# GaiYu0/dgl-1

Hardware: AMD Instinct MI355X
Metric: edges/sec on update_all g-SpMM (copy_u+sum, feat=128) (higher is better)
Workload: dtype fp32

## Files before the change

### dgl-1_amd/csrc/gspmm.hip

```cpp

#include "gspmm_impl.h"

namespace dglhip {

struct GatEpi {
  const float* a;
  const float* w;
  const float* dz;
  float alpha, lo, hi, scale;
  int apply_exp;
  float* rsum = nullptr;
  int hash_keep = 0;
  uint64_t seed = 0;
  const int64_t* seed_off = nullptr;
  uint32_t thr = 0;
  const float* el = nullptr;
  const float* er = nullptr;
};

__device__ __forceinline__ float gat_slope(const GatEpi& e, float a, int xpos) {
  if (xpos >= 0) return xpos ? 1.0f : e.alpha;
  return e.apply_exp ? (a <= 1.0f ? e.alpha : 1.0f) : (a <= 0.0f ? e.alpha : 1.0f);
}

// ... 441 lines not shown
  if (num_chunks > 0) {
    SumLaunch c{num_chunks, feat_len, elen, indptr, indices, eid, ufeat, efeat, partial,
                nullptr, chunk_beg, chunk_end, false, false, ufeat_ld};
    dispatch_sum(msg_op, false, c, stream);
  }
  if (num_light > 0) {
    SumLaunch l{num_light, feat_len, elen, indptr, indices, eid, ufeat, efeat, out,
                light_rows, nullptr, nullptr, accum,
                stream_output(num_light + num_heavy, feat_len), ufeat_ld};
    dispatch_sum(msg_op, mean, l, stream);
  }
  if (num_heavy > 0) {
    const int64_t blocks = (num_heavy + 3) / 4;
    auto combine = mean ? (accum ? gspmm_combine_kernel<true, true> : gspmm_combine_kernel<true, false>)
                        : (accum ? gspmm_combine_kernel<false, true> : gspmm_combine_kernel<false, false>);
    timed_launch(stream, [&] {
      hipLaunchKernelGGL(combine, grid_1d(blocks), dim3(256), 0, stream, num_heavy, feat_len,
                         indptr, heavy_rows, heavy_chunk_ptr, partial, out);
    });
  }
  API_END();
}

int dglhip_gspmm_items_columns_device(int msg_op, int64_t num_items, int64_t feat_len,
                                      const int32_t* item_rows, const int64_t* item_ptr,
                                      int accumulate, const int32_t* indices, const int64_t* eid,
                                      const float* ufeat, int64_t ufeat_ld, int64_t ufeat_rows,
                                      int items_per_wave, int column_parts, const float* efeat,
                                      int64_t efeat_len, float* out, void* stream_) {
  API_BEGIN();
  hipStream_t stream = static_cast<hipStream_t>(stream_);
  DGLHIP_CHECK(msg_op >= 0 && msg_op <= 3, "unknown msg op " << msg_op);
  DGLHIP_CHECK(num_items >= 0 && feat_len >= 0 && ufeat_rows >= 0, "negative size");
  DGLHIP_CHECK(items_per_wave == 1 || items_per_wave == 2,
               "items_per_wave " << items_per_wave << ": 1 or 2");
  DGLHIP_CHECK(column_parts == 1 || column_parts == 2,
               "column_parts " << column_parts << ": 1 or 2");
  if (num_items == 0 || feat_len == 0) return 0;
  DGLHIP_CHECK(item_rows && item_ptr && indices && out, "null items/indices/out");
  const int64_t elen = check_operands(msg_op, feat_len, ufeat, efeat, efeat_len);
  check_ufeat_ld(ufeat_ld, feat_len);
  SumLaunch a{num_items, feat_len, elen, nullptr, indices, eid, ufeat, efeat,
              out, item_rows, item_ptr, item_ptr + 1, accumulate != 0, false, ufeat_ld,
              ufeat_rows, items_per_wave, items_per_wave == 2 ? column_parts : 1};
  dispatch_sum(msg_op, false, a, stream);
  API_END();
}

int dglhip_gspmm_items_table_device(int msg_op, int64_t num_items, int64_t feat_len,
                                    const int32_t* item_rows, const int64_t* item_ptr,
                                    int accumulate, const int32_t* indices, const int64_t* eid,
                                    const float* ufeat, int64_t ufeat_ld, int64_t ufeat_rows,
                                    int items_per_wave, const float* efeat, int64_t efeat_len,
                                    float* out, void* stream_) {
  return dglhip_gspmm_items_columns_device(msg_op, num_items, feat_len, item_rows, item_ptr,
                                           accumulate, indices, eid, ufeat, ufeat_ld, ufeat_rows,
                                           items_per_wave, 1, efeat, efeat_len, out, stream_);
}

int dglhip_gspmm_items_device(int msg_op, int64_t num_items, int64_t feat_len,
                              const int32_t* item_rows, const int64_t* item_ptr, int accumulate,
                              const int32_t* indices, const int64_t* eid, const float* ufeat,
                              int64_t ufeat_ld, const float* efeat, int64_t efeat_len,
                              float* out, void* stream_) {
  return dglhip_gspmm_items_table_device(msg_op, num_items, feat_len, item_rows, item_ptr,
                                         accumulate, indices, eid, ufeat, ufeat_ld, 0, 1, efeat,
                                         efeat_len, out, stream_);
}

// ... 328 lines not shown
```

### dgl-1_amd/csrc/gspmm_impl.h

```cpp
#pragma once
#include <hip/hip_runtime.h>

#include <algorithm>
#include <cstdint>
#include <initializer_list>
#include <mutex>
#include <vector>

#include "../../include/dgl_hip.h"
#include "common.h"
#include "launch.h"
#include "timing.h"

namespace dglhip {

__host__ __device__ __forceinline__ uint32_t gat_mix32(uint32_t x) {
  x ^= x >> 16;
  x *= 0x7feb352du;
  x ^= x >> 15;
  x *= 0x846ca68bu;
  x ^= x >> 16;
  return x;
}

__host__ __device__ __forceinline__ bool gat_keep(uint64_t seed, int64_t idx, uint32_t thr) {
  const uint64_t i = static_cast<uint64_t>(idx);
  const uint32_t r = gat_mix32(gat_mix32(static_cast<uint32_t>(i) ^ static_cast<uint32_t>(seed)) ^
                               (static_cast<uint32_t>(i >> 32) + static_cast<uint32_t>(seed >> 32) +
                                0x9e3779b9u));
  return r >= thr;
}

static inline uint32_t gat_drop_threshold(float p) {
  const double t = static_cast<double>(p) * 4294967296.0;
  return t >= 4294967295.0 ? 0xffffffffu : static_cast<uint32_t>(t);
}

typedef float f32x2 __attribute__((ext_vector_type(2)));
typedef float f32x4 __attribute__((ext_vector_type(4)));

template <int VEC> struct Vec;
template <> struct Vec<1> {
  typedef float T;
  static __device__ __forceinline__ T zero() { return 0.0f; }
  static __device__ __forceinline__ T splat(float x) { return x; }
  static __device__ __forceinline__ T fma(T a, T b, T c) { return __builtin_fmaf(a, b, c); }
  static __device__ __forceinline__ T max(T a, T b) { return a > b ? a : b; }
};
template <> struct Vec<2> {
  typedef f32x2 T;
  static __device__ __forceinline__ T zero() { return T{0.0f, 0.0f}; }
  static __device__ __forceinline__ T splat(float x) { return T{x, x}; }
  static __device__ __forceinline__ T fma(T a, T b, T c) {
    return T{__builtin_fmaf(a.x, b.x, c.x), __builtin_fmaf(a.y, b.y, c.y)};
  }
};
template <> struct Vec<4> {
  typedef f32x4 T;
  static __device__ __forceinline__ T zero() { return T{0.0f, 0.0f, 0.0f, 0.0f}; }
// ... 385 lines not shown
      const int rb = nmax - k;
      u32x4 v[DEPTH];
#pragma unroll
      for (int j = 0; j < DEPTH; ++j) {
        if (j < rb)
          v[j] = __builtin_amdgcn_raw_buffer_load_b128(table, row_broadcast(ids, j) + lane_off,
                                                       0, 0);
      }
      if (k + DEPTH < nmax) ids = batch_ids(k + DEPTH);
#pragma unroll
      for (int j = 0; j < DEPTH; ++j) {
        if (j < rb) {
          const f32x4 sum = acc + *reinterpret_cast<const f32x4*>(&v[j]);
          acc = k + j < my_n ? sum : acc;
        }
      }
    }
  }
#pragma unroll
  for (int t = 0; t < 4; ++t)
    if (q == t && i0 + t < num_items) store_out<4, ACCUM ? 2 : 4>(out + r[t] * F, f0, acc);
}

template <bool MEAN, bool ACCUM>
__global__ __launch_bounds__(256) void gspmm_combine_kernel(
    int64_t num_heavy, int64_t F, const int64_t* __restrict__ indptr,
    const int32_t* __restrict__ heavy_rows, const int64_t* __restrict__ heavy_chunk_ptr,
    const float* __restrict__ partial, float* __restrict__ out) {
  const int64_t wave = block_linear() * (blockDim.x >> 6) + (threadIdx.x >> 6);
  if (wave >= num_heavy) return;
  const int lane = threadIdx.x & 63;
  const int64_t row = heavy_rows[wave];
  const int64_t c0 = heavy_chunk_ptr[wave], c1 = heavy_chunk_ptr[wave + 1];
  const float deg = static_cast<float>(indptr[row + 1] - indptr[row]);
  for (int64_t f = lane; f < F; f += 64) {
    float acc = (ACCUM && !MEAN) ? out[row * F + f] + partial[c0 * F + f] : partial[c0 * F + f];
    for (int64_t c = c0 + 1; c < c1; ++c) acc += partial[c * F + f];
    if (MEAN && deg > 1.0f) acc = acc / deg;
    if (MEAN && ACCUM) acc = out[row * F + f] + acc;
    out[row * F + f] = acc;
  }
}

__device__ __forceinline__ bool max_takes(float x, float best) {
  return (best == best) & !(x <= best);
}
// ... 130 lines not shown
  if (group < 64 && F >= 16) {
    vec = 1;
    group = 64;
  }
}

struct SumLaunch {
  int64_t num_items, F, elen;
  const int64_t* indptr;
  const int32_t* indices;
  const int64_t* eid;
  const float* ufeat;
  const float* efeat;
  float* out;
  const int32_t* row_order;
  const int64_t* chunk_beg;
  const int64_t* chunk_end;
  bool accumulate;
  bool nt_out = false;
  int64_t ldu = 0;
  int64_t urows = 0;
  int items_per_wave = 1;
  int column_parts = 1;
};

static inline bool stream_output(int64_t rows, int64_t feat_len) {
  return rows * feat_len * int64_t(sizeof(float)) > (int64_t(512) << 20);
}

static inline bool items_pair_applies(const SumLaunch& a) {
  const int64_t ldu = a.ldu ? a.ldu : a.F;
  return a.items_per_wave == 2 && a.F == 128 && a.urows > 0 && ldu % 4 == 0 &&
         reinterpret_cast<uintptr_t>(a.ufeat) % 16 == 0 &&
         reinterpret_cast<uintptr_t>(a.out) % 16 == 0 &&
         a.urows * ldu * int64_t(sizeof(float)) < (int64_t(1) << 32);
}

static inline bool items_columns_applies(const SumLaunch& a) {
  const int64_t ldu = a.ldu ? a.ldu : a.F;
  return a.column_parts == 2 && items_pair_applies(a) &&
         a.urows * ldu * int64_t(sizeof(float)) <= int64_t(0xfffffc00u);
}

static inline void launch_items_columns(const SumLaunch& a, hipStream_t stream) {
  constexpr int DEPTH = 12;
  const int64_t blocks = 2 * ((a.num_items + 15) / 16);
  DGLHIP_CHECK(blocks <= 0x7fffffff, "grid too large: " << blocks);
  const int64_t ldu = a.ldu ? a.ldu : a.F;
  auto kernel = a.accumulate ? gspmm_items_columns_kernel<DEPTH, true>
                             : gspmm_items_columns_kernel<DEPTH, false>;
  timed_launch(stream, [&] {
    hipLaunchKernelGGL(kernel, grid_1d(blocks), dim3(256), 0, stream, a.num_items, ldu,
                       static_cast<uint32_t>(a.urows * ldu * int64_t(sizeof(float))), a.indices,
                       a.ufeat, a.out, a.row_order, a.chunk_beg);
  });
}

static inline void launch_items_pair(const SumLaunch& a, hipStream_t stream) {
  constexpr int DEPTH = 10;
  const int64_t blocks = (a.num_items + 7) / 8;
  DGLHIP_CHECK(blocks <= 0x7fffffff, "grid too large: " << blocks);
  const int64_t ldu = a.ldu ? a.ldu : a.F;
  auto kernel = a.accumulate ? gspmm_items_pair_kernel<DEPTH, true>
                             : gspmm_items_pair_kernel<DEPTH, false>;
  timed_launch(stream, [&] {
    hipLaunchKernelGGL(kernel, grid_1d(blocks), dim3(256), 0, stream, a.num_items, ldu,
                       static_cast<uint32_t>(a.urows * ldu * int64_t(sizeof(float))), a.indices,
                       a.ufeat, a.out, a.row_order, a.chunk_beg);
  });
}

template <int VEC, int GROUP, int MSG, int EM, bool MEAN>
static inline void launch_sum(const SumLaunch& a, hipStream_t stream) {
  constexpr int UNROLL = 16;
  constexpr int ITEMS_PER_BLOCK = 4 * (64 / GROUP);
  const int64_t blocks = (a.num_items + ITEMS_PER_BLOCK - 1) / ITEMS_PER_BLOCK;
  DGLHIP_CHECK(blocks <= 0x7fffffff, "grid too large: " << blocks);
  if (blocks == 0) return;
  const bool chunked = a.chunk_beg != nullptr;
  auto kernel = gspmm_sum_kernel<VEC, GROUP, UNROLL, MSG, EM, MEAN, false, false>;
  if (chunked && a.accumulate)
    kernel = gspmm_sum_kernel<VEC, GROUP, UNROLL, MSG, EM, MEAN, true, true>;
  else if (chunked)
    kernel = gspmm_sum_kernel<VEC, GROUP, UNROLL, MSG, EM, MEAN, true, false>;
  else if (a.accumulate)
    kernel = gspmm_sum_kernel<VEC, GROUP, UNROLL, MSG, EM, MEAN, false, true>;
  constexpr bool POL_OK = MSG == DGLHIP_MSG_COPY_U && VEC == 2 && GROUP == 64 && !MEAN;
  if constexpr (POL_OK) {
    if (chunked && a.row_order && !a.nt_out) {
      if (items_columns_applies(a)) {
        launch_items_columns(a, stream);
        return;
      }
      if (items_pair_applies(a)) {
        launch_items_pair(a, stream);
        return;
      }
      if (a.accumulate)
        kernel = gspmm_sum_kernel<VEC, GROUP, UNROLL, MSG, EM, false, true, true, POL_DEFAULT,
                                  true, 2>;
      else
        kernel = gspmm_sum_kernel<VEC, GROUP, UNROLL, MSG, EM, false, true, false, POL_DEFAULT,
                                  true, 4>;
    } else if (a.nt_out && !a.accumulate) {
      if (chunked)
        kernel = gspmm_sum_kernel<VEC, GROUP, UNROLL, MSG, EM, false, true, false, POL_NT_OUT>;
      else
        kernel = gspmm_sum_kernel<VEC, GROUP, UNROLL, MSG, EM, false, false, false, POL_NT_OUT>;
    }
  }
  timed_launch(stream, [&] {
    hipLaunchKernelGGL(kernel, grid_1d(blocks), dim3(256), 0, stream, a.num_items, a.F, a.elen,
// ... 95 lines not shown
```

### dgl-1_amd/csrc/spmm_plan.cc

```cpp
#include "spmm_plan.h"

#include <hip/hip_runtime.h>

#include <algorithm>
#include <climits>
#include <cmath>
#include <cstdlib>
#include <cstring>
#include <numeric>
#include <string>

#include "../../include/dgl_hip.h"
#include "common.h"

namespace dglhip {

namespace {

constexpr int64_t kRefWaves = 7168;
constexpr int64_t kCriticalMin = 16384;
constexpr int64_t kCutNum = 7168, kCutDen = 12000;
constexpr int64_t kChunkMin = 1024;

void hip_ok(hipError_t e, const char* what) {
  DGLHIP_CHECK(e == hipSuccess, what << ": " << hipGetErrorString(e));
}

std::string env_str(const char* name, const char* dflt) {
  const char* v = std::getenv(name);
  return v ? std::string(v) : std::string(dflt);
}

SpmmPolicy policy_from_env() {
  SpmmPolicy p;
  const std::string rs = env_str("DGLHIP_ROW_SPLIT", "auto");
  if (rs == "auto") p.row_split = -1;
  else if (rs == "off" || rs == "0" || rs.empty() || rs == "none" || rs == "None") p.row_split = 0;
  else p.row_split = std::stoll(rs);
  p.blocked = env_str("DGLHIP_BLOCKED", "auto") != "off";
  p.block_bytes = std::stoll(env_str("DGLHIP_BLOCK_BYTES", "6291456"));
  p.block_min_slots = std::stoll(env_str("DGLHIP_BLOCK_MIN_SLOTS", "12"));
  p.block_max_stretch = std::stod(env_str("DGLHIP_BLOCK_MAX_STRETCH", "3"));
  p.short_rows = env_str("DGLHIP_SHORT_ROWS", "on") != "off";
  p.pad_rows = env_str("DGLHIP_PAD_ROWS", "auto") == "auto";
  p.items_per_wave = env_str("DGLHIP_ITEMS_PER_WAVE", "2") == "1" ? 1 : 2;
  p.column_parts = env_str("DGLHIP_COLUMN_PARTS", "2") == "1" ? 1 : 2;
  return p;
}

std::mutex g_pol_mu;
SpmmPolicy& pol_ref() {
  static SpmmPolicy p = policy_from_env();
  return p;
}

double lines_per_row(int64_t F, int64_t ld) {
  int64_t tot = 0;
  for (int64_t u = 0; u < 32; ++u) {
    const int64_t off = (u * ld * 4) % 128;
    tot += (off + 4 * F + 127) / 128;
  }
  return tot / 32.0;
}

inline int64_t cdiv(int64_t a, int64_t b) { return (a + b - 1) / b; }

inline bool copies_u(int msg) {
  return msg == DGLHIP_MSG_COPY_U || msg == DGLHIP_MSG_COPY_U_BF16;
}
// ... 28 lines not shown
    const char* bb = std::getenv("DGLHIP_SWEEP_BLOCK_BYTES");
    if (bb && std::atoll(bb) >= (int64_t(1) << 20)) q.block_bytes = std::atoll(bb);
    return q;
  }();
  return p;
}
}

SweepPolicy sweep_policy() {
  std::lock_guard<std::mutex> lk(g_pol_mu);
  return sweep_ref();
}

void set_spmm_policy(const SpmmPolicy& p) {
  DGLHIP_CHECK(p.block_bytes > 0 && p.block_min_slots >= 1 && p.block_max_stretch > 0 &&
                   p.block_table_min >= 0 && p.block_table_max >= p.block_table_min &&
                   p.block_max_suffix >= 0 && p.tier_min_rows >= 0 && p.pad_min_bytes >= 0,
               "invalid g-SpMM schedule policy");
  DGLHIP_CHECK(p.row_split >= -1, "row_split: -1 auto, 0 off or a chunk length");
  DGLHIP_CHECK(p.items_per_wave == 1 || p.items_per_wave == 2,
               "items_per_wave " << p.items_per_wave << ": 1 or 2");
  DGLHIP_CHECK(p.column_parts == 1 || p.column_parts == 2,
               "column_parts " << p.column_parts << ": 1 or 2");
  std::lock_guard<std::mutex> lk(g_pol_mu);
  pol_ref() = p;
}

int64_t split_threshold(const SpmmPolicy& p, int64_t nnz, int64_t max_degree, int64_t waves) {
  if (p.row_split == 0) return 0;
  if (p.row_split < 0) {
    const int64_t R = std::max<int64_t>(waves, 2);
    const int64_t t = std::max<int64_t>(4096, nnz * kCutNum / (kCutDen * R));
    return max_degree > std::max<int64_t>(kCriticalMin, nnz / (R / 2)) ? t : 0;
  }
  return max_degree > p.row_split ? p.row_split : 0;
}

int64_t padded_width(int64_t F) {
  int64_t best = F;
  double best_lines = lines_per_row(F, F);
  for (int64_t ld : {cdiv(F, 16) * 16, cdiv(F, 32) * 32}) {
    if (ld > F && ld % 2 == 0) {
      const double l = lines_per_row(F, ld);
      if (l < best_lines * 0.95 && l < lines_per_row(F, best) - 1e-9) {
        best = ld;
        best_lines = l;
// ... 615 lines not shown
};

enum Path { PATH_HOST = 0, PATH_ROWS = 1, PATH_BLOCKED = 2, PATH_MAX_BLOCKED = 3, PATH_SWEEP = 4 };

int g_blocked_mean_add = [] {
  const char* e = std::getenv("DGLHIP_BLOCKED_MEAN_ADD");
  return e && *e ? std::atoi(e) : 1;
}();

inline bool blocked_mean_add() { return g_blocked_mean_add != 0; }

struct Decision {
  Path path = PATH_ROWS;
  std::shared_ptr<BlockedPlan> bp;
  std::shared_ptr<Cuts> cuts;
  std::shared_ptr<SweepPlan> sw;
  bool pad = false;
  int64_t ld = 0;
  int64_t split = 0;
  int64_t ws_pad = 0, ws_vals = 0, ws_map = 0, ws_partial = 0;
  int64_t ws_sums = 0;
  int items_per_wave = 1;
  int column_parts = 1;
  int64_t total() const { return ws_pad + ws_vals + ws_map + ws_partial + ws_sums; }
};

inline int64_t align256(int64_t b) { return (b + 255) / 256 * 256; }

bool pad_rows(const SpmmPolicy& p, int msg, int red, int64_t F, int64_t urows) {
  return p.pad_rows && (msg == DGLHIP_MSG_COPY_U || msg == DGLHIP_MSG_U_MUL_E) &&
         (red == DGLHIP_REDUCE_SUM || red == DGLHIP_REDUCE_MEAN || accum(red)) &&
         urows * F * 4 >= p.pad_min_bytes && padded_width(F) != F;
}

void check_args(const SpmmPlan& plan, const RunArgs& a) {
  DGLHIP_CHECK(a.msg >= 0 && a.msg <= 3, "unknown msg op " << a.msg);
  DGLHIP_CHECK(a.red >= 0 && a.red <= 4, "unknown reduce op " << a.red);
  DGLHIP_CHECK(a.F >= 0, "negative feat_len");
  DGLHIP_CHECK(a.emode >= DGLHIP_EDGE_BY_SLOT && a.emode <= DGLHIP_EDGE_BY_MAP,
               "unknown edge layout " << a.emode);
  DGLHIP_CHECK(a.ldu == 0 || a.ldu == a.F || (a.ldu > a.F && a.ldu % 2 == 0),
               "ufeat_ld " << a.ldu << ": 0, feat_len, or an even width > feat_len");
  DGLHIP_CHECK(a.ldu <= a.F || (a.msg == DGLHIP_MSG_COPY_U || a.msg == DGLHIP_MSG_U_MUL_E),
               "row-strided source rows: copy_u or u_mul_e");
  DGLHIP_CHECK(a.ldu <= a.F || a.red != DGLHIP_REDUCE_MAX, "row-strided source rows: not max");
  const bool use_u = a.msg != DGLHIP_MSG_COPY_E;
// ... 26 lines not shown
  if ((a.red == DGLHIP_REDUCE_SUM || a.red == DGLHIP_REDUCE_MEAN ||
       a.red == DGLHIP_REDUCE_SUM_ACCUM) && a.msg == DGLHIP_MSG_COPY_U &&
      a.ufeat && !a.efeat && !strided && a.F == 128) {
    d.sw = plan.sweep(a.F * 4,
                      a.red == DGLHIP_REDUCE_SUM_ACCUM ? 2 : (a.red == DGLHIP_REDUCE_MEAN ? 1 : 0),
                      s);
    if (d.sw) {
      d.path = PATH_SWEEP;
      return d;
    }
  }
  const bool mean_add = blocked_mean_add() && a.red == DGLHIP_REDUCE_MEAN_ACCUM &&
                        a.msg == DGLHIP_MSG_COPY_U && !a.efeat;
  if ((sumlike || mean_add) && a.ufeat &&
      ((cu && !a.efeat) || (a.msg == DGLHIP_MSG_U_MUL_E && a.efeat))) {
    d.bp = plan.blocked(ld_in * elem, p.block_bytes, s);
    if (d.bp) {
      d.path = PATH_BLOCKED;
      const auto lh = plan.span(s);
      const double slice = static_cast<double>(lh.second - lh.first) * ld_in * elem / d.bp->B;
      const double reach = p.column_parts == 2 ? 3.0 : 1.5;
      d.items_per_wave = p.items_per_wave == 2 && slice <= reach * p.block_bytes ? 2 : 1;
      d.column_parts = d.items_per_wave == 2 ? p.column_parts : 1;
      if (mean_add) d.ws_sums = align256(plan.num_rows() * a.F * 4);
      if (!strided && fp32u && pad_rows(p, a.msg, DGLHIP_REDUCE_SUM, a.F, a.urows)) {
        d.pad = true;
        d.ld = padded_width(a.F);
        d.ws_pad = align256(a.urows * d.ld * 4);
      } else {
        d.ld = strided ? a.ldu : 0;
      }
      if (a.msg == DGLHIP_MSG_U_MUL_E) {
        if (a.elen == 1) d.ws_vals = align256(plan.nnz() * 4);
        if (a.emode == DGLHIP_EDGE_BY_MAP) d.ws_map = align256(plan.nnz() * 8);
      }
      return d;
    }
  }
  if (a.red == DGLHIP_REDUCE_MAX && a.ufeat && !strided && fp32u &&
      (a.msg == DGLHIP_MSG_COPY_U ||
       (a.msg == DGLHIP_MSG_U_MUL_E &&
        (a.emode == DGLHIP_EDGE_BY_SLOT ||
         (a.emode == DGLHIP_EDGE_BY_EID && plan.eid_identity(a.erow, s)))))) {
    d.cuts = plan.cuts(a.F * 4, p.block_bytes, s);
    if (d.cuts) {
      d.path = PATH_MAX_BLOCKED;
// ... 95 lines not shown
    const int64_t* erows = nullptr;
    if (a.msg == DGLHIP_MSG_U_MUL_E) {
      const int64_t* rows = nullptr;
      if (a.emode == DGLHIP_EDGE_BY_SLOT) {
        rows = plan.plan_pos64(bp, s);
      } else if (a.emode == DGLHIP_EDGE_BY_EID) {
        rows = plan.eid_identity(a.erow, s) ? plan.plan_pos64(bp, s)
                                            : plan.plan_eidmap(bp, a.erow, s);
      } else {
        int64_t* m = reinterpret_cast<int64_t*>(ws.take(d.ws_map));
        plan_compose_device(plan.nnz(), bp.pos.data<int32_t>(), a.erow, m, s);
        rows = m;
      }
      if (a.elen == 1) {
        float* v = reinterpret_cast<float*>(ws.take(d.ws_vals));
        plan_gather_vals_device(plan.nnz(), rows, a.efeat, v, s);
        ev = v;
      } else {
        erows = rows;
      }
    }
    for (size_t i = 0; i < bp.launches.size(); ++i) {
      const BlockItems& it = bp.launches[i];
      DGLHIP_CHECK(dglhip_gspmm_items_columns_device(
                       a.msg, it.n_items, a.F, it.rows.data<int32_t>(), it.ptr.data<int64_t>(),
                       (i == 0 && first_writes) ? 0 : 1, bp.indices.data<int32_t>(),
                       ev ? nullptr : erows, static_cast<const float*>(uf), d.ld, a.urows,
                       d.items_per_wave, d.column_parts,
                       ev ? ev : (a.msg == DGLHIP_MSG_U_MUL_E ? a.efeat : nullptr),
                       elen, sums, s) == 0,
                   DGLGetLastError());
    }
    if (a.red == DGLHIP_REDUCE_MEAN) plan_div_degree_device(plan.num_rows(), a.F, plan.indptr(),
                                                            a.out, s);
    if (d.ws_sums) plan_add_mean_device(plan.num_rows(), a.F, plan.indptr(), sums, a.out, s);
    return;
  }
  if (d.path == PATH_MAX_BLOCKED) {
    const Cuts& c = *d.cuts;
    const int64_t* base = c.data.data<int64_t>();
    const int64_t* eid = nullptr;
    for (int64_t b = 0; b + 1 < c.n; ++b) {
      DGLHIP_CHECK(dglhip_gspmm_max_ranges_device(
                       a.msg, plan.num_rows(), a.F, plan.indptr(), base + b * plan.num_rows(),
                       base + (b + 1) * plan.num_rows(), b ? 1 : 0, plan.indices(), eid,
                       static_cast<const float*>(uf), a.efeat, a.elen, a.out, a.arg,
                       plan.row_order(), s) == 0,
                   DGLGetLastError());
    }
    return;
  }
// ... 152 lines not shown
  *accum_per_cu = p.accum_per_cu;
  API_END();
}

int dglhip_spmm_get_policy(DGLHipSpmmPolicy* out) {
  API_BEGIN();
  DGLHIP_CHECK(out != nullptr, "null pointer argument");
  const SpmmPolicy p = spmm_policy();
  out->row_split = p.row_split;
  out->blocked = p.blocked;
  out->short_rows = p.short_rows;
  out->pad_rows = p.pad_rows;
  out->items_per_wave = p.items_per_wave;
  out->block_bytes = p.block_bytes;
  out->block_table_min = p.block_table_min;
  out->block_table_max = p.block_table_max;
  out->block_min_slots = p.block_min_slots;
  out->block_max_stretch = p.block_max_stretch;
  out->block_max_suffix = p.block_max_suffix;
  out->block_min_row_bytes = p.block_min_row_bytes;
  out->tier_min_rows = p.tier_min_rows;
  out->pad_min_bytes = p.pad_min_bytes;
  out->column_parts = p.column_parts;
  out->reserved = 0;
  API_END();
}

int dglhip_spmm_set_policy(const DGLHipSpmmPolicy* in) {
  API_BEGIN();
  DGLHIP_CHECK(in != nullptr, "null pointer argument");
  SpmmPolicy p;
  p.row_split = in->row_split;
  p.blocked = in->blocked != 0;
  p.short_rows = in->short_rows != 0;
  p.pad_rows = in->pad_rows != 0;
  p.items_per_wave = in->items_per_wave;
  p.block_bytes = in->block_bytes;
  p.block_table_min = in->block_table_min;
  p.block_table_max = in->block_table_max;
  p.block_min_slots = in->block_min_slots;
  p.block_max_stretch = in->block_max_stretch;
  p.block_max_suffix = in->block_max_suffix;
  p.block_min_row_bytes = in->block_min_row_bytes;
  p.tier_min_rows = in->tier_min_rows;
  p.pad_min_bytes = in->pad_min_bytes;
  p.column_parts = in->column_parts;
  set_spmm_policy(p);
  API_END();
}

int dglhip_spmm_split_threshold(int64_t nnz, int64_t max_degree, int64_t waves, int64_t* out) {
  API_BEGIN();
  DGLHIP_CHECK(out != nullptr, "null pointer argument");
  *out = split_threshold(spmm_policy(), nnz, max_degree, waves > 0 ? waves : kRefWaves);
  API_END();
}

int dglhip_spmm_padded_width(int64_t feat_len, int64_t* out) {
  API_BEGIN();
  DGLHIP_CHECK(out != nullptr && feat_len >= 1, "bad argument");
  *out = padded_width(feat_len);
  API_END();
}

int dglhip_spmm_plan_create(int device_type, int device_id, int64_t num_rows, int64_t num_cols,
                            int64_t nnz, const int64_t* indptr, const int32_t* indices,
                            const int64_t* host_indptr, const int32_t* row_order, void* stream,
                            DGLHipSpmmPlan* out) {
  API_BEGIN();
// ... 85 lines not shown
```

### dgl-1_amd/csrc/spmm_plan.h

```cpp
#pragma once

#include <hip/hip_runtime.h>

#include <cstdint>
#include <map>
#include <memory>
#include <mutex>
#include <tuple>
#include <vector>

#include "runtime.h"

namespace dglhip {

struct SpmmPolicy {
  int64_t row_split = -1;
  int blocked = 1;
  int short_rows = 1;
  int pad_rows = 1;
  int items_per_wave = 2;
  int64_t block_bytes = 6 << 20;
  int64_t block_table_min = 16 << 20;
  int64_t block_table_max = 256 << 20;
  int64_t block_min_slots = 12;
  double block_max_stretch = 3.0;
  double block_max_suffix = 1.0 / 16;
  int64_t block_min_row_bytes = 128;
  int64_t tier_min_rows = 1 << 16;
  int64_t pad_min_bytes = 4 << 20;
  int column_parts = 2;
};

SpmmPolicy spmm_policy();
void set_spmm_policy(const SpmmPolicy& p);

int64_t split_threshold(const SpmmPolicy& p, int64_t nnz, int64_t max_degree, int64_t waves);

int64_t padded_width(int64_t F);

struct BlockItems {
  rt::NDArray rows;
  rt::NDArray ptr;
  int64_t n_items = 0, nnz = 0, off = 0;
  bool suffix = false;
};

struct BlockedPlan {
  int B = 0;
  bool has_suffix = false;
  std::vector<BlockItems> launches;
  rt::NDArray indices;
  rt::NDArray pos;
  rt::NDArray absent;
// ... 181 lines not shown
```

### dgl-1_amd/dgl/_ffi.py

```python
from __future__ import absolute_import

import ctypes
import os

import torch

from .base import DGLError

__all__ = ["LIB", "check_call", "lib_path", "tensor_arg", "call_packed", "list_global_names",
           "PackedFunction", "get_global_func", "CAPINamespace"]

_HERE = os.path.dirname(os.path.abspath(__file__))
_LIBNAME = "libdgl_hip.so"


def lib_path():
    cands = []
    env = os.environ.get("DGL_LIBRARY_PATH")
    if env:
        for d in env.split(os.pathsep):
            cands.append(os.path.join(d, _LIBNAME) if os.path.isdir(d) else d)
    cands.append(os.path.join(os.path.dirname(_HERE), "lib", _LIBNAME))
    for c in cands:
        if os.path.isfile(c):
# ... 102 lines not shown
        "dglhip_gat_logits_device": (_c_int, [_c_i64] * 3 + [_vp] * 6),
        "dglhip_gat_logits_host": (_c_int, [_c_i64] * 3 + [_vp] * 5 + [_c_int]),
        "dglhip_set_gat_logit_recompute": (_c_int, [_c_int]),
        "dglhip_gat_aggregate_ranges_device": (_c_int, [_c_i64, _c_i64, _c_i64, _c_i64, _vp,
                                                        _vp, _c_int, _vp, _vp, _vp, _vp, _vp,
                                                        ctypes.c_float, ctypes.c_float,
                                                        ctypes.c_float, _c_int, ctypes.c_float,
                                                        ctypes.c_uint64, _vp, _vp, _vp, _vp, _vp,
                                                        _vp]),
        "dglhip_set_gat_variant": (_c_int, [_c_int]),
        "dglhip_set_gat_bwd_variant": (_c_int, [_c_int]),
        "dglhip_gat_attention_grad_device": (_c_int, [_c_i64, _c_i64, _c_i64, _vp, _vp, _vp, _vp,
                                                      _vp, _vp, _vp, ctypes.c_float,
                                                      ctypes.c_float, ctypes.c_float, _c_int,
                                                      ctypes.c_float, _vp, _vp]),
        "dglhip_gspmm_items_device": (_c_int, [_c_int, _c_i64, _c_i64, _vp, _vp, _c_int, _vp, _vp,
                                               _vp, _c_i64, _vp, _c_i64, _vp, _vp]),
        "dglhip_gspmm_items_table_device": (_c_int, [_c_int, _c_i64, _c_i64, _vp, _vp, _c_int,
                                                     _vp, _vp, _vp, _c_i64, _c_i64, _c_int, _vp,
                                                     _c_i64, _vp, _vp]),
        "dglhip_gspmm_items_columns_device": (_c_int, [_c_int, _c_i64, _c_i64, _vp, _vp, _c_int,
                                                       _vp, _vp, _vp, _c_i64, _c_i64, _c_int,
                                                       _c_int, _vp, _c_i64, _vp, _vp]),
        "dglhip_gspmm_sweep_device": (_c_int, [_c_i64, _c_i64, _vp, _vp, _vp, _vp, _vp, _c_i64,
                                               _c_i64, _c_int, _c_int, _c_int, _vp]),
        "dglhip_gspmm_sweep_stream_geometry": (_c_int, [_c_int, _c_int, _vp]),
        "dglhip_set_sweep_per_cu": (_c_int, [_c_int]),
        "dglhip_sweep_barrier_expiries": (_c_int, [_c_int, _vp]),
        "dglhip_set_sweep_rows": (_c_int, [_c_int]),
        "dglhip_get_sweep_rows": (_c_int, [_vp]),
        "dglhip_set_sweep_schedule": (_c_int, [_c_int, _c_i64, _c_i64, _c_int, _c_int, _c_i64,
                                               _c_i64, _c_int]),
        "dglhip_get_sweep_schedule": (_c_int, [_vp, _vp, _vp, _vp, _vp, _vp, _vp, _vp]),
        "dglhip_set_gat_fwd_waves": (_c_int, [_c_int]),
        "dglhip_set_sweep_unroll": (_c_int, [_c_int]),
        "dglhip_gspmm_sweep_stream_device": (_c_int, [_c_i64, _c_i64, _vp, _vp, _c_int, _vp, _vp,
                                                      _vp, _vp, _vp, _c_int, _c_int, _c_int, _vp,
                                                      _c_i64, _c_int, _c_int, _vp]),
        "dglhip_gspmm_max_ranges_device": (_c_int, [_c_int, _c_i64, _c_i64, _vp, _vp, _vp, _c_int,
                                                    _vp, _vp, _vp, _vp, _c_i64, _vp, _vp, _vp,
                                                    _vp]),
        "dglhip_gsddmm_ranges_device": (_c_int, [_c_int, _c_i64, _c_i64, _c_i64, _vp, _vp, _vp,
                                                 _vp, _vp, _vp, _vp, _vp, _vp]),
        "dglhip_gat_attention_grad_ranges_device": (_c_int, [_c_i64, _c_i64, _c_i64, _vp, _vp,
                                                             _vp, _vp, _vp, _vp, _vp, _vp, _vp,
                                                             ctypes.c_float, ctypes.c_float,
# ... 324 lines not shown
```

### dgl-1_amd/dgl/kernel.py

```python
from __future__ import absolute_import

import contextlib
import ctypes
import os
import weakref

import numpy as np
import torch

from . import _ffi, _handoff
from ._ffi import LIB, check_call, ptr
from .base import DGLError

__all__ = ["CSR", "SparseAdj", "build_csr", "gspmm", "gsddmm_dot",
           "MSG_COPY_U", "MSG_U_MUL_E", "MSG_COPY_E", "RED_SUM", "RED_MAX", "RED_MEAN"]

MSG_COPY_U, MSG_U_MUL_E, MSG_COPY_E = 0, 1, 2
MSG_COPY_U_BF16 = 3
RED_SUM, RED_MAX, RED_MEAN = 0, 1, 2
RED_SUM_ACCUM = 3
RED_MEAN_ACCUM = 4
_ACCUM = (RED_SUM_ACCUM, RED_MEAN_ACCUM)
ORDER_EID, ORDER_COL = 0, 1
SLOT = "slot"

_MSG_NAMES = {"copy_src": MSG_COPY_U, "copy_u": MSG_COPY_U, "src_mul_edge": MSG_U_MUL_E,
              "u_mul_e": MSG_U_MUL_E, "copy_edge": MSG_COPY_E, "copy_e": MSG_COPY_E}
_RED_NAMES = {"sum": RED_SUM, "max": RED_MAX, "mean": RED_MEAN}



_REF_WAVES = 7168
_WAVES = {}


class _Policy(ctypes.Structure):
    _fields_ = [("row_split", ctypes.c_int64), ("blocked", ctypes.c_int32),
                ("short_rows", ctypes.c_int32), ("pad_rows", ctypes.c_int32),
                ("items_per_wave", ctypes.c_int32), ("block_bytes", ctypes.c_int64),
                ("block_table_min", ctypes.c_int64), ("block_table_max", ctypes.c_int64),
                ("block_min_slots", ctypes.c_int64), ("block_max_stretch", ctypes.c_double),
                ("block_max_suffix", ctypes.c_double), ("block_min_row_bytes", ctypes.c_int64),
                ("tier_min_rows", ctypes.c_int64), ("pad_min_bytes", ctypes.c_int64),
                ("column_parts", ctypes.c_int32), ("reserved", ctypes.c_int32)]


_POLICY_KEYS = tuple(n for n, _ in _Policy._fields_ if n != "reserved")
_POLICY_GEN = [0]


def schedule_policy():
    p = _Policy()
    check_call(LIB.dglhip_spmm_get_policy(ctypes.addressof(p)))
    return {k: getattr(p, k) for k in _POLICY_KEYS}


def set_schedule_policy(**changes):
    p = _Policy()
    check_call(LIB.dglhip_spmm_get_policy(ctypes.addressof(p)))
    old = {k: getattr(p, k) for k in _POLICY_KEYS}
    for k, v in changes.items():
        if k not in _POLICY_KEYS:
            raise DGLError("unknown schedule policy field %r" % (k,))
        setattr(p, k, v)
    check_call(LIB.dglhip_spmm_set_policy(ctypes.addressof(p)))
    _POLICY_GEN[0] += 1
    return old


@contextlib.contextmanager
# ... 2274 lines not shown
```

### include/dgl_hip.h

```cpp
#ifndef DGL_HIP_H_
#define DGL_HIP_H_

#include <stddef.h>
#include <stdint.h>

#ifdef __cplusplus
extern "C" {
#endif

#define DGLHIP_ABI_VERSION 1


const char* DGLGetLastError(void);
void DGLAPISetLastError(const char* msg);
int dglhip_abi_version(void);
const char* dglhip_build_info(void);


#define DGLHIP_ORDER_EID 0
#define DGLHIP_ORDER_COL 1

int dglhip_coo_to_csr_host(int64_t num_rows, int64_t num_cols, int64_t nnz,
                           const int64_t* row, const int64_t* col, int order,
                           int64_t* indptr, int32_t* indices, int64_t* eid);
// ... 71 lines not shown
                                   int64_t ufeat_ld, void* stream);

typedef struct DGLHipSpmmPlanObj* DGLHipSpmmPlan;

#define DGLHIP_EDGE_BY_SLOT 0
#define DGLHIP_EDGE_BY_EID 1
#define DGLHIP_EDGE_BY_MAP 2

typedef struct {
  int64_t row_split;
  int32_t blocked;
  int32_t short_rows;
  int32_t pad_rows;
  int32_t items_per_wave;
  int64_t block_bytes;
  int64_t block_table_min, block_table_max;
  int64_t block_min_slots;
  double block_max_stretch;
  double block_max_suffix;
  int64_t block_min_row_bytes;
  int64_t tier_min_rows;
  int64_t pad_min_bytes;
  int32_t column_parts;
  int32_t reserved;
} DGLHipSpmmPolicy;
int dglhip_spmm_get_policy(DGLHipSpmmPolicy* out);
int dglhip_spmm_set_policy(const DGLHipSpmmPolicy* policy);
int dglhip_spmm_split_threshold(int64_t nnz, int64_t max_degree, int64_t waves, int64_t* out);
int dglhip_spmm_padded_width(int64_t feat_len, int64_t* out);

int dglhip_spmm_plan_create(int device_type, int device_id, int64_t num_rows, int64_t num_cols,
                            int64_t nnz, const int64_t* indptr, const int32_t* indices,
                            const int64_t* host_indptr, const int32_t* row_order, void* stream,
                            DGLHipSpmmPlan* out);
int dglhip_spmm_plan_free(DGLHipSpmmPlan plan);
int dglhip_spmm_plan_workspace(DGLHipSpmmPlan plan, int msg_op, int reduce_op, int64_t feat_len,
                               int64_t ufeat_ld, int64_t num_src_rows, int64_t efeat_len,
                               int edge_layout, const int64_t* erow, void* stream, int64_t* bytes);
int dglhip_spmm_plan_run(DGLHipSpmmPlan plan, int msg_op, int reduce_op, int64_t feat_len,
                         const void* ufeat, int64_t ufeat_ld, int64_t num_src_rows,
                         const float* efeat, int64_t efeat_len, int edge_layout,
                         const int64_t* erow, float* out, int64_t* arg_out, void* workspace,
                         int64_t workspace_bytes, void* stream);
#define DGLHIP_PLAN_PATH_HOST 0
#define DGLHIP_PLAN_PATH_ROWS 1
#define DGLHIP_PLAN_PATH_BLOCKED 2
#define DGLHIP_PLAN_PATH_MAX_BLOCKED 3
// ... 184 lines not shown
                                const int32_t* row_order, const float* el, const float* er,
                                const float* ft, float alpha, float clamp_lo, float clamp_hi,
                                int apply_exp, float drop_p, uint64_t seed,
                                const int64_t* seed_offset, float* out_ft, float* out_z,
                                float* attn_out, float* attn_drop_out, void* stream);

int dglhip_gspmm_items_device(int msg_op, int64_t num_items, int64_t feat_len,
                              const int32_t* item_rows, const int64_t* item_ptr, int accumulate,
                              const int32_t* indices, const int64_t* eid, const float* ufeat,
                              int64_t ufeat_ld, const float* efeat, int64_t efeat_len,
                              float* out, void* stream);
int dglhip_gspmm_items_table_device(int msg_op, int64_t num_items, int64_t feat_len,
                                    const int32_t* item_rows, const int64_t* item_ptr,
                                    int accumulate, const int32_t* indices, const int64_t* eid,
                                    const float* ufeat, int64_t ufeat_ld, int64_t ufeat_rows,
                                    int items_per_wave, const float* efeat, int64_t efeat_len,
                                    float* out, void* stream);
int dglhip_gspmm_items_columns_device(int msg_op, int64_t num_items, int64_t feat_len,
                                      const int32_t* item_rows, const int64_t* item_ptr,
                                      int accumulate, const int32_t* indices, const int64_t* eid,
                                      const float* ufeat, int64_t ufeat_ld, int64_t ufeat_rows,
                                      int items_per_wave, int column_parts, const float* efeat,
                                      int64_t efeat_len, float* out, void* stream);

int dglhip_gspmm_sweep_device(int64_t num_rows, int64_t feat_len, const int64_t* indptr,
                              const int32_t* indices, const float* ufeat, float* out,
                              const int32_t* row_order, int64_t col_lo, int64_t block_cols,
                              int num_blocks, int mean, int rows_per_wave, void* stream);

int dglhip_gspmm_sweep_stream_geometry(int rows_per_wave, int per_cu, int64_t* waves_per_launch);
int dglhip_gspmm_sweep_stream_geometry_mode(int rows_per_wave, int per_cu, int mode,
                                            int64_t* waves_per_launch);
int dglhip_gspmm_sweep_stream_device(int64_t num_rows, int64_t waves_total,
                                     const int32_t* row_order, const int32_t* counts,
                                     int num_blocks, const int64_t* seg_beg, const int32_t* lay,
                                     const int64_t* indptr, const float* ufeat, float* out,
                                     int mode, int rows_per_wave, int per_cu, int* arrive,
                                     int64_t arrive_len, int lag, int max_spin, void* stream);
int dglhip_set_blocked_mean_add(int on);
int dglhip_set_sweep_schedule(int on, int64_t table_min, int64_t block_bytes, int lag,
                              int max_spin, int64_t accum_table_min, int64_t accum_min_slots,
                              int accum_per_cu);
int dglhip_get_sweep_schedule(int* on, int64_t* table_min, int64_t* block_bytes, int* lag,
                              int* max_spin, int64_t* accum_table_min,
                              int64_t* accum_min_slots, int* accum_per_cu);
int dglhip_sweep_barrier_expiries(int reset, int64_t* out);
// ... 312 lines not shown
```

Baseline: 40.25 billion.

## Add quarter-column items kernel with eight rows per wave and DPP id broadcast

```diff
diff --git a/dgl-1_amd/csrc/gspmm.hip b/dgl-1_amd/csrc/gspmm.hip
--- a/dgl-1_amd/csrc/gspmm.hip
+++ b/dgl-1_amd/csrc/gspmm.hip
@@ -487,29 +487,45 @@
   API_END();
 }
 
+int dglhip_gspmm_items_quarters_device(int msg_op, int64_t num_items, int64_t feat_len,
+                                       const int32_t* item_rows, const int64_t* item_ptr,
+                                       int accumulate, const int32_t* indices, const int64_t* eid,
+                                       const float* ufeat, int64_t ufeat_ld, int64_t ufeat_rows,
+                                       int items_per_wave, int column_parts, int column_quarters,
+                                       const float* efeat, int64_t efeat_len, float* out,
+                                       void* stream_) {
+  API_BEGIN();
+  hipStream_t stream = static_cast<hipStream_t>(stream_);
+  DGLHIP_CHECK(msg_op >= 0 && msg_op <= 3, "unknown msg op " << msg_op);
+  DGLHIP_CHECK(num_items >= 0 && feat_len >= 0 && ufeat_rows >= 0, "negative size");
+  DGLHIP_CHECK(items_per_wave == 1 || items_per_wave == 2,
+               "items_per_wave " << items_per_wave << ": 1 or 2");
+  DGLHIP_CHECK(column_parts == 1 || column_parts == 2,
+               "column_parts " << column_parts << ": 1 or 2");
+  DGLHIP_CHECK(column_quarters == 0 || column_quarters == 1,
+               "column_quarters " << column_quarters << ": 0 or 1");
+  if (num_items == 0 || feat_len == 0) return 0;
+  DGLHIP_CHECK(item_rows && item_ptr && indices && out, "null items/indices/out");
+  const int64_t elen = check_operands(msg_op, feat_len, ufeat, efeat, efeat_len);
+  check_ufeat_ld(ufeat_ld, feat_len);
+  SumLaunch a{num_items, feat_len, elen, nullptr, indices, eid, ufeat, efeat,
+              out, item_rows, item_ptr, item_ptr + 1, accumulate != 0, false, ufeat_ld,
+              ufeat_rows, items_per_wave, items_per_wave == 2 ? column_parts : 1,
+              items_per_wave == 2 && column_parts == 2 ? column_quarters : 0};
+  dispatch_sum(msg_op, false, a, stream);
+  API_END();
+}
+
 int dglhip_gspmm_items_columns_device(int msg_op, int64_t num_items, int64_t feat_len,
                                       const int32_t* item_rows, const int64_t* item_ptr,
                                       int accumulate, const int32_t* indices, const int64_t* eid,
                                       const float* ufeat, int64_t ufeat_ld, int64_t ufeat_rows,
                                       int items_per_wave, int column_parts, const float* efeat,
                                       int64_t efeat_len, float* out, void* stream_) {
-  API_BEGIN();
-  hipStream_t stream = static_cast<hipStream_t>(stream_);
-  DGLHIP_CHECK(msg_op >= 0 && msg_op <= 3, "unknown msg op " << msg_op);
-  DGLHIP_CHECK(num_items >= 0 && feat_len >= 0 && ufeat_rows >= 0, "negative size");
-  DGLHIP_CHECK(items_per_wave == 1 || items_per_wave == 2,
-               "items_per_wave " << items_per_wave << ": 1 or 2");
-  DGLHIP_CHECK(column_parts == 1 || column_parts == 2,
-               "column_parts " << column_parts << ": 1 or 2");
-  if (num_items == 0 || feat_len == 0) return 0;
-  DGLHIP_CHECK(item_rows && item_ptr && indices && out, "null items/indices/out");
-  const int64_t elen = check_operands(msg_op, feat_len, ufeat, efeat, efeat_len);
-  check_ufeat_ld(ufeat_ld, feat_len);
-  SumLaunch a{num_items, feat_len, elen, nullptr, indices, eid, ufeat, efeat,
-              out, item_rows, item_ptr, item_ptr + 1, accumulate != 0, false, ufeat_ld,
-              ufeat_rows, items_per_wave, items_per_wave == 2 ? column_parts : 1};
-  dispatch_sum(msg_op, false, a, stream);
-  API_END();
+  return dglhip_gspmm_items_quarters_device(msg_op, num_items, feat_len, item_rows, item_ptr,
+                                            accumulate, indices, eid, ufeat, ufeat_ld, ufeat_rows,
+                                            items_per_wave, column_parts, 0, efeat, efeat_len,
+                                            out, stream_);
 }
 
 int dglhip_gspmm_items_table_device(int msg_op, int64_t num_items, int64_t feat_len,
diff --git a/dgl-1_amd/csrc/gspmm_impl.h b/dgl-1_amd/csrc/gspmm_impl.h
--- a/dgl-1_amd/csrc/gspmm_impl.h
+++ b/dgl-1_amd/csrc/gspmm_impl.h
@@ -35,6 +35,13 @@
   const double t = static_cast<double>(p) * 4294967296.0;
   return t >= 4294967295.0 ? 0xffffffffu : static_cast<uint32_t>(t);
 }
+
+#ifndef DGLHIP_QUARTERS_DEPTH
+#define DGLHIP_QUARTERS_DEPTH 8
+#endif
+#ifndef DGLHIP_QUARTERS_IDW
+#define DGLHIP_QUARTERS_IDW 4
+#endif
 
 typedef float f32x2 __attribute__((ext_vector_type(2)));
 typedef float f32x4 __attribute__((ext_vector_type(4)));
@@ -466,6 +473,145 @@
     if (q == t && i0 + t < num_items) store_out<4, ACCUM ? 2 : 4>(out + r[t] * F, f0, acc);
 }
 
+__device__ __forceinline__ uint32_t group_broadcast(uint32_t v, int j) {
+  switch (j) {
+#define DGLHIP_GROUP_BCAST(J)                                                              \
+  case J: {                                                                                \
+    const uint32_t lo = __builtin_amdgcn_update_dpp(0, v, 0x150 + J, 0xf, 0xf, true);      \
+    return __builtin_amdgcn_update_dpp(lo, v, 0x158 + J, 0xf, 0xc, true);                  \
+  }
+    DGLHIP_GROUP_BCAST(0) DGLHIP_GROUP_BCAST(1) DGLHIP_GROUP_BCAST(2) DGLHIP_GROUP_BCAST(3)
+    DGLHIP_GROUP_BCAST(4) DGLHIP_GROUP_BCAST(5) DGLHIP_GROUP_BCAST(6)
+    default: {
+      const uint32_t lo = __builtin_amdgcn_update_dpp(0, v, 0x157, 0xf, 0xf, true);
+      return __builtin_amdgcn_update_dpp(lo, v, 0x15f, 0xf, 0xc, true);
+    }
+#undef DGLHIP_GROUP_BCAST
+  }
+}
+
+template <int DEPTH, int IDW, bool ACCUM>
+__global__ __launch_bounds__(256) void gspmm_items_quarters_kernel(
+    int64_t num_items, int64_t ldu, uint32_t table_bytes,
+    const int32_t* __restrict__ indices, const float* __restrict__ ufeat,
+    float* __restrict__ out, const int32_t* __restrict__ item_rows,
+    const int64_t* __restrict__ item_ptr) {
+  constexpr int WIN = 8 * IDW;
+  constexpr int NB = WIN / DEPTH;
+  static_assert(IDW >= 1 && IDW <= 4 && NB >= 1 && NB * DEPTH == WIN && DEPTH % IDW == 0,
+                "a window of ids is a whole number of batches, a batch whole lanes of it");
+  typedef unsigned int u32x4 __attribute__((ext_vector_type(4)));
+  constexpr int64_t F = 128;
+  constexpr uint32_t kOff = 0xfffffc00u;
+  const int lane = threadIdx.x & 63;
+  const int g = lane >> 3, gl = lane & 7;
+  const int64_t bl = block_linear();
+  const int quarter = static_cast<int>(bl % 8) & 3;
+  const int64_t wave =
+      (bl >> 2) * (blockDim.x >> 6) +
+      __builtin_amdgcn_readfirstlane(static_cast<int>(threadIdx.x >> 6));
+  const int64_t i0 = wave * 8;
+  if (i0 >= num_items) return;
+  int64_t p[9];
+#pragma unroll
+  for (int t = 0; t < 9; ++t) p[t] = item_ptr[i0 + t < num_items ? i0 + t : num_items];
+  const bool owns = i0 + g < num_items;
+  const int32_t my_row = item_rows[owns ? i0 + g : num_items - 1];
+  int nmin = static_cast<int>(p[1] - p[0]), nmax = nmin;
+  int my_n = nmin, my_rel = 0;
+#pragma unroll
+  for (int t = 1; t < 8; ++t) {
+    const int n = static_cast<int>(p[t + 1] - p[t]);
+    nmin = min(nmin, n);
+    nmax = max(nmax, n);
+    my_n = g == t ? n : my_n;
+    my_rel = g == t ? static_cast<int>(p[t] - p[0]) : my_rel;
+  }
+  const int32_t* __restrict__ idx = indices + p[0];
+  const uint32_t ld4 = static_cast<uint32_t>(ldu) * 4u;
+  const uint32_t lane_off =
+      static_cast<uint32_t>(quarter) * 128u + static_cast<uint32_t>(gl) * 16u;
+  const __amdgpu_buffer_rsrc_t table = __builtin_amdgcn_make_buffer_rsrc(
+      const_cast<float*>(ufeat), 0, static_cast<int>(table_bytes), 0x00020000);
+  const int64_t f0 = int64_t(quarter) * 32 + int64_t(gl) * 4;
+
+  const int64_t ahead = item_ptr[num_items] - p[0];
+  const int room = static_cast<int>(ahead < 0x7fffffff ? ahead : 0x7fffffff);
+
+  auto load_ids = [&](int w, uint32_t (&ids)[IDW]) {
+    const int first = w + gl * IDW;
+    uint32_t raw[IDW];
+#pragma unroll
+    for (int i = 0; i < IDW; ++i) raw[i] = 0;
+    if (first < my_n) {
+      const int s0 = my_rel + first;
+      if (s0 + IDW <= room) {
+        __builtin_memcpy(raw, idx + s0, sizeof(raw));
+      } else {
+#pragma unroll
+        for (int i = 0; i < IDW; ++i) raw[i] = static_cast<uint32_t>(idx[min(s0 + i, room - 1)]);
+      }
+    }
+#pragma unroll
+    for (int i = 0; i < IDW; ++i) ids[i] = first + i < my_n ? raw[i] * ld4 : kOff;
+  };
+  auto slot_off = [&](const uint32_t (&ids)[IDW], int s) -> uint32_t {
+    return group_broadcast(ids[s % IDW], s / IDW) + lane_off;
+  };
+
+  f32x4 acc = Vec<4>::zero();
+  if (ACCUM && owns) acc = load_out<4, 2>(out + int64_t(my_row) * F, f0);
+  if (nmax > 0) {
+    uint32_t ids[IDW];
+    load_ids(0, ids);
+    int k = 0, left = NB;
+    auto next_ids = [&]() {
+      if (k + DEPTH >= nmax) return;
+      if (--left > 0) {
+#pragma unroll
+        for (int i = 0; i < IDW; ++i)
+          ids[i] = __builtin_amdgcn_update_dpp(0, ids[i], 0x100 + DEPTH / IDW, 0xf, 0xf, true);
+      } else {
+        load_ids(k + DEPTH, ids);
+        left = NB;
+      }
+    };
+#pragma unroll 1
+    for (; k + DEPTH <= nmin; k += DEPTH) {
+      u32x4 v[DEPTH];
+#pragma unroll
+      for (int j = 0; j < DEPTH; ++j)
+        v[j] = __builtin_amdgcn_raw_buffer_load_b128(table, slot_off(ids, j), 0, 0);
+      next_ids();
+#pragma unroll
+      for (int j = 0; j < DEPTH; ++j) acc += *reinterpret_cast<const f32x4*>(&v[j]);
+    }
+#pragma unroll 1
+    for (; k < nmax; k += DEPTH) {
+      const int rb = nmax - k;
+      u32x4 v[DEPTH];
+#pragma unroll
+      for (int j = 0; j < DEPTH; ++j) {
+        if (j < rb)
+          v[j] = __builtin_amdgcn_raw_buffer_load_b128(table, slot_off(ids, j), 0, 0);
+      }
+      next_ids();
+#pragma unroll
+      for (int j = 0; j < DEPTH; ++j) {
+        if (j < rb) {
+          const f32x4 sum = acc + *reinterpret_cast<const f32x4*>(&v[j]);
+          acc = k + j < my_n ? sum : acc;
+        }
+      }
+    }
+  }
+#pragma unroll
+  for (int t = 0; t < 8; ++t) {
+    const int64_t row = __builtin_amdgcn_readlane(my_row, 8 * t);
+    if (g == t && i0 + t < num_items) store_out<4, ACCUM ? 2 : 4>(out + row * F, f0, acc);
+  }
+}
+
 template <bool MEAN, bool ACCUM>
 __global__ __launch_bounds__(256) void gspmm_combine_kernel(
     int64_t num_heavy, int64_t F, const int64_t* __restrict__ indptr,
@@ -642,6 +788,7 @@
   int64_t urows = 0;
   int items_per_wave = 1;
   int column_parts = 1;
+  int column_quarters = 0;
 };
 
 static inline bool stream_output(int64_t rows, int64_t feat_len) {
@@ -669,6 +816,24 @@
   const int64_t ldu = a.ldu ? a.ldu : a.F;
   auto kernel = a.accumulate ? gspmm_items_columns_kernel<DEPTH, true>
                              : gspmm_items_columns_kernel<DEPTH, false>;
+  timed_launch(stream, [&] {
+    hipLaunchKernelGGL(kernel, grid_1d(blocks), dim3(256), 0, stream, a.num_items, ldu,
+                       static_cast<uint32_t>(a.urows * ldu * int64_t(sizeof(float))), a.indices,
+                       a.ufeat, a.out, a.row_order, a.chunk_beg);
+  });
+}
+
+static inline bool items_quarters_applies(const SumLaunch& a) {
+  return a.column_quarters == 1 && items_columns_applies(a);
+}
+
+static inline void launch_items_quarters(const SumLaunch& a, hipStream_t stream) {
+  constexpr int DEPTH = DGLHIP_QUARTERS_DEPTH, IDW = DGLHIP_QUARTERS_IDW;
+  const int64_t blocks = 4 * ((a.num_items + 31) / 32);
+  DGLHIP_CHECK(blocks <= 0x7fffffff, "grid too large: " << blocks);
+  const int64_t ldu = a.ldu ? a.ldu : a.F;
+  auto kernel = a.accumulate ? gspmm_items_quarters_kernel<DEPTH, IDW, true>
+                             : gspmm_items_quarters_kernel<DEPTH, IDW, false>;
   timed_launch(stream, [&] {
     hipLaunchKernelGGL(kernel, grid_1d(blocks), dim3(256), 0, stream, a.num_items, ldu,
                        static_cast<uint32_t>(a.urows * ldu * int64_t(sizeof(float))), a.indices,
@@ -708,6 +873,10 @@
   constexpr bool POL_OK = MSG == DGLHIP_MSG_COPY_U && VEC == 2 && GROUP == 64 && !MEAN;
   if constexpr (POL_OK) {
     if (chunked && a.row_order && !a.nt_out) {
+      if (items_quarters_applies(a)) {
+        launch_items_quarters(a, stream);
+        return;
+      }
       if (items_columns_applies(a)) {
         launch_items_columns(a, stream);
         return;
diff --git a/dgl-1_amd/csrc/spmm_plan.cc b/dgl-1_amd/csrc/spmm_plan.cc
--- a/dgl-1_amd/csrc/spmm_plan.cc
+++ b/dgl-1_amd/csrc/spmm_plan.cc
@@ -45,6 +45,7 @@
   p.pad_rows = env_str("DGLHIP_PAD_ROWS", "auto") == "auto";
   p.items_per_wave = env_str("DGLHIP_ITEMS_PER_WAVE", "2") == "1" ? 1 : 2;
   p.column_parts = env_str("DGLHIP_COLUMN_PARTS", "2") == "1" ? 1 : 2;
+  p.column_quarters = env_str("DGLHIP_COLUMN_QUARTERS", "1") == "0" ? 0 : 1;
   return p;
 }
 
@@ -119,6 +120,10 @@
                "items_per_wave " << p.items_per_wave << ": 1 or 2");
   DGLHIP_CHECK(p.column_parts == 1 || p.column_parts == 2,
                "column_parts " << p.column_parts << ": 1 or 2");
+  DGLHIP_CHECK(p.column_quarters == 0 || p.column_quarters == 1,
+               "column_quarters " << p.column_quarters << ": 0 or 1");
+  DGLHIP_CHECK(p.column_quarters_min_bytes >= 0,
+               "column_quarters_min_bytes " << p.column_quarters_min_bytes << ": negative");
   std::lock_guard<std::mutex> lk(g_pol_mu);
   pol_ref() = p;
 }
@@ -780,6 +785,7 @@
   int64_t ws_sums = 0;
   int items_per_wave = 1;
   int column_parts = 1;
+  int column_quarters = 0;
   int64_t total() const { return ws_pad + ws_vals + ws_map + ws_partial + ws_sums; }
 };
 
@@ -852,6 +858,8 @@
       const double reach = p.column_parts == 2 ? 3.0 : 1.5;
       d.items_per_wave = p.items_per_wave == 2 && slice <= reach * p.block_bytes ? 2 : 1;
       d.column_parts = d.items_per_wave == 2 ? p.column_parts : 1;
+      d.column_quarters = d.column_parts == 2 && p.column_quarters == 1 &&
+                          slice / 2 >= static_cast<double>(p.column_quarters_min_bytes);
       if (mean_add) d.ws_sums = align256(plan.num_rows() * a.F * 4);
       if (!strided && fp32u && pad_rows(p, a.msg, DGLHIP_REDUCE_SUM, a.F, a.urows)) {
         d.pad = true;
@@ -993,11 +1001,11 @@
     }
     for (size_t i = 0; i < bp.launches.size(); ++i) {
       const BlockItems& it = bp.launches[i];
-      DGLHIP_CHECK(dglhip_gspmm_items_columns_device(
+      DGLHIP_CHECK(dglhip_gspmm_items_quarters_device(
                        a.msg, it.n_items, a.F, it.rows.data<int32_t>(), it.ptr.data<int64_t>(),
                        (i == 0 && first_writes) ? 0 : 1, bp.indices.data<int32_t>(),
                        ev ? nullptr : erows, static_cast<const float*>(uf), d.ld, a.urows,
-                       d.items_per_wave, d.column_parts,
+                       d.items_per_wave, d.column_parts, d.column_quarters,
                        ev ? ev : (a.msg == DGLHIP_MSG_U_MUL_E ? a.efeat : nullptr),
                        elen, sums, s) == 0,
                    DGLGetLastError());
@@ -1196,7 +1204,8 @@
   out->tier_min_rows = p.tier_min_rows;
   out->pad_min_bytes = p.pad_min_bytes;
   out->column_parts = p.column_parts;
-  out->reserved = 0;
+  out->column_quarters = p.column_quarters;
+  out->column_quarters_min_bytes = p.column_quarters_min_bytes;
   API_END();
 }
 
@@ -1219,6 +1228,8 @@
   p.tier_min_rows = in->tier_min_rows;
   p.pad_min_bytes = in->pad_min_bytes;
   p.column_parts = in->column_parts;
+  p.column_quarters = in->column_quarters;
+  p.column_quarters_min_bytes = in->column_quarters_min_bytes;
   set_spmm_policy(p);
   API_END();
 }
diff --git a/dgl-1_amd/csrc/spmm_plan.h b/dgl-1_amd/csrc/spmm_plan.h
--- a/dgl-1_amd/csrc/spmm_plan.h
+++ b/dgl-1_amd/csrc/spmm_plan.h
@@ -29,6 +29,8 @@
   int64_t tier_min_rows = 1 << 16;
   int64_t pad_min_bytes = 4 << 20;
   int column_parts = 2;
+  int column_quarters = 1;
+  int64_t column_quarters_min_bytes = 5 << 20;
 };
 
 SpmmPolicy spmm_policy();
diff --git a/dgl-1_amd/dgl/_ffi.py b/dgl-1_amd/dgl/_ffi.py
--- a/dgl-1_amd/dgl/_ffi.py
+++ b/dgl-1_amd/dgl/_ffi.py
@@ -148,6 +148,9 @@
         "dglhip_gspmm_items_columns_device": (_c_int, [_c_int, _c_i64, _c_i64, _vp, _vp, _c_int,
                                                        _vp, _vp, _vp, _c_i64, _c_i64, _c_int,
                                                        _c_int, _vp, _c_i64, _vp, _vp]),
+        "dglhip_gspmm_items_quarters_device": (_c_int, [_c_int, _c_i64, _c_i64, _vp, _vp, _c_int,
+                                                        _vp, _vp, _vp, _c_i64, _c_i64, _c_int,
+                                                        _c_int, _c_int, _vp, _c_i64, _vp, _vp]),
         "dglhip_gspmm_sweep_device": (_c_int, [_c_i64, _c_i64, _vp, _vp, _vp, _vp, _vp, _c_i64,
                                                _c_i64, _c_int, _c_int, _c_int, _vp]),
         "dglhip_gspmm_sweep_stream_geometry": (_c_int, [_c_int, _c_int, _vp]),
diff --git a/dgl-1_amd/dgl/kernel.py b/dgl-1_amd/dgl/kernel.py
--- a/dgl-1_amd/dgl/kernel.py
+++ b/dgl-1_amd/dgl/kernel.py
@@ -42,10 +42,11 @@
                 ("block_min_slots", ctypes.c_int64), ("block_max_stretch", ctypes.c_double),
                 ("block_max_suffix", ctypes.c_double), ("block_min_row_bytes", ctypes.c_int64),
                 ("tier_min_rows", ctypes.c_int64), ("pad_min_bytes", ctypes.c_int64),
-                ("column_parts", ctypes.c_int32), ("reserved", ctypes.c_int32)]
-
-
-_POLICY_KEYS = tuple(n for n, _ in _Policy._fields_ if n != "reserved")
+                ("column_parts", ctypes.c_int32), ("column_quarters", ctypes.c_int32),
+                ("column_quarters_min_bytes", ctypes.c_int64)]
+
+
+_POLICY_KEYS = tuple(n for n, _ in _Policy._fields_)
 _POLICY_GEN = [0]
 
 
diff --git a/include/dgl_hip.h b/include/dgl_hip.h
--- a/include/dgl_hip.h
+++ b/include/dgl_hip.h
@@ -117,7 +117,8 @@
   int64_t tier_min_rows;
   int64_t pad_min_bytes;
   int32_t column_parts;
-  int32_t reserved;
+  int32_t column_quarters;
+  int64_t column_quarters_min_bytes;
 } DGLHipSpmmPolicy;
 int dglhip_spmm_get_policy(DGLHipSpmmPolicy* out);
 int dglhip_spmm_set_policy(const DGLHipSpmmPolicy* policy);
@@ -348,6 +349,13 @@
                                       const float* ufeat, int64_t ufeat_ld, int64_t ufeat_rows,
                                       int items_per_wave, int column_parts, const float* efeat,
                                       int64_t efeat_len, float* out, void* stream);
+int dglhip_gspmm_items_quarters_device(int msg_op, int64_t num_items, int64_t feat_len,
+                                       const int32_t* item_rows, const int64_t* item_ptr,
+                                       int accumulate, const int32_t* indices, const int64_t* eid,
+                                       const float* ufeat, int64_t ufeat_ld, int64_t ufeat_rows,
+                                       int items_per_wave, int column_parts, int column_quarters,
+                                       const float* efeat, int64_t efeat_len, float* out,
+                                       void* stream);
 
 int dglhip_gspmm_sweep_device(int64_t num_rows, int64_t feat_len, const int64_t* indptr,
                               const int32_t* indices, const float* ufeat, float* out,
```

Measured after the change: 40.31 billion (median of 6 runs). Within noise of the previous version (+0.1%).
